# Anton-Le/PhysicsBasedBayesianInference

Hardware: AMD Instinct MI355X
Metric: leapfrog-steps*chains/sec (node); d=128 Gaussian, ensemble=65536 (higher is better)
Workload: dtype f64; 1 GPU; C2: d=128 dense-precision Gaussian, fp64, L=10 leapfrog steps per HMC iteration, in-kernel Philox momentum + Metropolis; chains_per_gpu=65536, total_chains=65536, D=128, L=10, parallelism=ensemble-sharded x1, draw=f32 (single-precision Box-Muller on the transcendental unit; momenta only)

## Files before the change

### physicsbasedbayesianinference_amd/csrc/kernels_dense_dev.h

```cpp
#pragma once
#include <cstdlib>
#include <vector>

#include "pbbi_buf.h"
#include <type_traits>

#include "pbbi_internal.h"
#include "pbbi_rng.h"

namespace {

typedef double v4f64 __attribute__((ext_vector_type(4)));
typedef double v2f64 __attribute__((ext_vector_type(2)));

constexpr int BLOCK = 256;
constexpr int CHAINS_PER_WAVE = 16;
constexpr int CHAINS_PER_WG = 64;

#ifdef PBBI_STAMPS
static unsigned long long* g_stamp_buf = nullptr;
extern "C" void pbbi_debug_set_stamp_buffer(void* p) { g_stamp_buf = (unsigned long long*)p; }
#if PBBI_STAMPS == 2
#define STAMP(i)                                                                      \
    do {                                                                              \
        if (((i) == 0 || (i) == 41) && prm.stamps && lane == 0) {                     \
            unsigned long long t_;                                                    \
            asm volatile("s_memrealtime %0\n\ts_waitcnt lgkmcnt(0)" : "=s"(t_)::"memory"); \
            prm.stamps[((size_t)blockIdx.x * 8 + wave) * 64 + (i)] = t_;              \
        }                                                                             \
    } while (0)
#else
#define STAMP(i)                                                                      \
    do {                                                                              \
        if (prm.stamps && lane == 0) {                                                \
            __builtin_amdgcn_sched_barrier(0);                                        \
            unsigned long long t_;                                                    \
            asm volatile("s_memtime %0\n\ts_waitcnt lgkmcnt(0)" : "=s"(t_)::"memory"); \
            prm.stamps[((size_t)blockIdx.x * 8 + wave) * 64 + (i)] = t_;              \
            __builtin_amdgcn_sched_barrier(0);                                        \
        }                                                                             \
    } while (0)
#endif
#else
#define STAMP(i) do { } while (0)
#endif

struct DensePrm {
#ifdef PBBI_STAMPS
    unsigned long long* stamps;
#endif
    const double* frag;
    const double* mu;
    const double* q_in;
    const double* p_in;
    const double* u_in;
    const double* mass;
    double* q_out;
    double* p_out;
    double* v_out;
    double* ratio_out;
    uint8_t* reject_out;
    int64_t N, ldn_in, ldn_out;
    double h, cst, kT;
    int L, D, flags, rng, mode;
    uint64_t seed, iter, chain0;
    const int32_t* steps_in;
    int32_t* steps_out;
    double* carry_g;
    uint8_t* carry_sel;
    uint32_t carry_slab_bytes;
    int fuse_S, fuse_wrap2, fuse_first;
    int64_t fuse_slab0, fuse_slab;
    double* fuse_q_base;
};

template <int NT>
__device__ __forceinline__ void stage_lds(const double* __restrict__ gfrag,
                                          const double* __restrict__ gmu, v2f64* frag2,
                                          double* mu) {
    constexpr int DP = 16 * NT;
    const v2f64* src = reinterpret_cast<const v2f64*>(gfrag);
    for (int i = threadIdx.x; i < DP * DP / 2; i += BLOCK) frag2[i] = src[i];
    for (int i = threadIdx.x; i < DP; i += BLOCK) mu[i] = gmu[i];
    __syncthreads();
}

template <int NT>
__device__ __forceinline__ void matvec(const v2f64* __restrict__ fragL,
                                       const double* __restrict__ muG,
                                       const double (&q)[4 * NT], v4f64 (&acc)[NT]) {
    constexpr int KS = 4 * NT;
    constexpr int H = NT / 2;
    v2f64 A[H], An[H];
    double m0 = muG[0], mn = 0.0;
#pragma unroll
    for (int t2 = 0; t2 < H; ++t2) A[t2] = fragL[t2 * 64];
#pragma unroll
    for (int t = 0; t < NT; ++t) acc[t] = v4f64{0.0, 0.0, 0.0, 0.0};
#pragma unroll
    for (int s = 0; s < KS; ++s) {
        if (s + 1 < KS) {
#pragma unroll
            for (int t2 = 0; t2 < H; ++t2) An[t2] = fragL[((s + 1) * H + t2) * 64];
            mn = muG[4 * (s + 1)];
        }
        const double x = q[s] - m0;
#pragma unroll
        for (int t2 = 0; t2 < H; ++t2) {
            acc[2 * t2] = __builtin_amdgcn_mfma_f64_16x16x4f64(A[t2].x, x, acc[2 * t2], 0, 0, 0);
            acc[2 * t2 + 1] = __builtin_amdgcn_mfma_f64_16x16x4f64(A[t2].y, x, acc[2 * t2 + 1], 0, 0, 0);
        }
        __builtin_amdgcn_sched_barrier(0);
#pragma unroll
        for (int t2 = 0; t2 < H; ++t2) A[t2] = An[t2];
        m0 = mn;
    }
}

__device__ __forceinline__ double chain_sum(double x) {
    x += __shfl_xor(x, 16, 64);
    x += __shfl_xor(x, 32, 64);
    return x;
}

template <int NT>
__device__ __forceinline__ double dot_x_acc(const double* __restrict__ muG,
                                             const double (&q)[4 * NT], const v4f64 (&acc)[NT]) {
    double sum = 0.0;
#pragma unroll
    for (int t = 0; t < NT; ++t)
#pragma unroll
        for (int r = 0; r < 4; ++r) {
            const int s = 4 * t + r;
            sum += (q[s] - muG[4 * s]) * acc[t][r];
        }
    return sum;
}

template <bool FULL>
__device__ __forceinline__ double load_elem(__amdgpu_buffer_rsrc_t base, uint32_t voff,
                                            uint32_t stride4, uint32_t ld, int s, int g, int D) {
    if constexpr (FULL) return buf_load<double>(base, voff, (uint32_t)s * stride4);
    double val = 0.0;
    if (4 * s + 3 < D) {
        val = buf_load<double>(base, voff, (uint32_t)s * stride4);
    } else if (4 * s < D) {
        const bool ok = 4 * s + g < D;
        const double t = buf_load<double>(base, voff - (ok ? 0u : (uint32_t)g * ld),
                                          (uint32_t)s * stride4);
        val = ok ? t : 0.0;
    }
    return val;
}

template <bool FULL>
__device__ __forceinline__ void store_elem(__amdgpu_buffer_rsrc_t base, uint32_t voff,
                                           uint32_t stride4, int s, int g, int D, double val) {
    if constexpr (FULL) {
        buf_store(base, voff, (uint32_t)s * stride4, val);
        return;
    }
    if (4 * s + 3 < D) {
        buf_store(base, voff, (uint32_t)s * stride4, val);
    } else if (4 * s < D) {
        if (4 * s + g < D) buf_store(base, voff, (uint32_t)s * stride4, val);
    }
}

__device__ __forceinline__ double load_row(__amdgpu_buffer_rsrc_t base, uint32_t voff, uint32_t stride4, int s) {
    return buf_load<double>(base, voff, (uint32_t)s * stride4);
}
__device__ __forceinline__ void store_row(__amdgpu_buffer_rsrc_t base, uint32_t voff, uint32_t stride4, int s,
                                          double val) {
    buf_store(base, voff, (uint32_t)s * stride4, val);
}
template <bool FULL>
__device__ __forceinline__ __amdgpu_buffer_rsrc_t rows_of(const double* arr, int64_t n0, int D, int64_t ld,
                                                          int64_t N) {
    if constexpr (FULL) return buf_make(arr + n0);
    return buf_make_rows(arr + n0, D, ld, N, n0, 8);
}

template <int NT, int METHOD, bool FULL>
__global__ void __launch_bounds__(BLOCK, 1) k_dense_traj(DensePrm prm) {
    constexpr int DP = 16 * NT;
    constexpr int KS = 4 * NT;
    extern __shared__ __attribute__((aligned(16))) char smem[];
    v2f64* frag2 = reinterpret_cast<v2f64*>(smem);
    double* mu = reinterpret_cast<double*>(smem + (size_t)DP * DP * sizeof(double));
    stage_lds<NT>(prm.frag, prm.mu, frag2, mu);

    const int lane = threadIdx.x & 63;
    const int wave = __builtin_amdgcn_readfirstlane(threadIdx.x >> 6);
    const int g = lane >> 4;
    const int c = lane & 15;
    const v2f64* fragL = frag2 + lane;
    const double* muG = mu + g;
    const int D = prm.D;
    const bool unit = (prm.mass == nullptr);
    const double h = prm.h, h2 = prm.h * prm.h;
    const int64_t n_wg_tiles = (prm.N + CHAINS_PER_WG - 1) / CHAINS_PER_WG;

    for (int64_t wt = blockIdx.x; wt < n_wg_tiles; wt += gridDim.x) {
        const int64_t n0 = (wt * 4 + wave) * CHAINS_PER_WAVE;
        if (n0 >= prm.N) continue;
        const int64_t left = prm.N - n0;
        const bool valid = c < left;
        const int cc = c < left ? c : (int)left - 1;
        const uint32_t ld_in = 8u * (uint32_t)prm.ldn_in, ld_out = 8u * (uint32_t)prm.ldn_out;
        const uint32_t vin = (uint32_t)g * ld_in + 8u * (uint32_t)cc, s4in = 4u * ld_in;
        const uint32_t vout = (uint32_t)g * ld_out + 8u * (uint32_t)cc, s4out = 4u * ld_out;
        const __amdgpu_buffer_rsrc_t qin = buf_make(prm.q_in + n0);
        const __amdgpu_buffer_rsrc_t pin = buf_make(prm.p_in + n0);
        const __amdgpu_buffer_rsrc_t qout = buf_make(prm.q_out + n0);
        const __amdgpu_buffer_rsrc_t pout = buf_make(prm.p_out + n0);
        const bool have_pout = (prm.p_out != nullptr);
        const double m = unit ? 1.0 : prm.mass[n0 + cc];
        const uint64_t chain = prm.chain0 + (uint64_t)(n0 + cc);

        double q[KS], v[KS], a[KS];
        v4f64 acc[NT];
        double u = 0.0;
        if (prm.rng) {
            const double pstd = sqrt(m * prm.kT);
#pragma unroll
            for (int k = 0; k < KS / 4; ++k) {
                double z[4];
                rng_normal4d(prm.seed, PBBI_STREAM_MOMENTUM, prm.iter, chain, (uint32_t)((k << 2) | g),
                             (prm.flags & PBBI_DRAW_F64) != 0, z);
#pragma unroll
                for (int sl = 0; sl < 4; ++sl)
                    v[4 * k + sl] = (FULL || 16 * k + 4 * sl + g < D) ? z[sl] * pstd : 0.0;
            }
            u = rng_uniform(prm.seed, prm.iter, chain);
            if (have_pout && !(prm.flags & PBBI_COMPAT_P_FROM_OLDQ) && valid) {
#pragma unroll
                for (int s = 0; s < KS; ++s) store_elem<FULL>(pout, vout, s4out, s, g, D, v[s]);
            }
        } else {
#pragma unroll
            for (int s = 0; s < KS; ++s) v[s] = load_elem<FULL>(pin, vin, s4in, ld_in, s, g, D);
            if (prm.mode == 0) u = prm.u_in[n0 + cc];
        }
#pragma unroll
        for (int s = 0; s < KS; ++s) q[s] = load_elem<FULL>(qin, vin, s4in, ld_in, s, g, D);
        double pp_old = 0.0;
#pragma unroll
        for (int s = 0; s < KS; ++s) pp_old += v[s] * v[s];
        if (!unit) {
#pragma unroll
            for (int s = 0; s < KS; ++s) v[s] = v[s] / m;
        }

        matvec<NT>(fragL, muG, q, acc);
        double xg_old = dot_x_acc<NT>(muG, q, acc);
        double xg_new = xg_old;
#pragma unroll
        for (int t = 0; t < NT; ++t)
#pragma unroll
            for (int r = 0; r < 4; ++r) a[4 * t + r] = unit ? -acc[t][r] : -acc[t][r] / m;

        if constexpr (METHOD == PBBI_LEAPFROG) {
            for (int j = 0; j < prm.L; ++j) {
#pragma unroll
                for (int s = 0; s < KS; ++s) q[s] += (v[s] * h + (0.5 * a[s]) * h2);
                matvec<NT>(fragL, muG, q, acc);
                if (j == prm.L - 1) xg_new = dot_x_acc<NT>(muG, q, acc);
#pragma unroll
                for (int t = 0; t < NT; ++t)
#pragma unroll
                    for (int r = 0; r < 4; ++r) {
                        const int s = 4 * t + r;
                        const double an = unit ? -acc[t][r] : -acc[t][r] / m;
                        v[s] += (0.5 * (a[s] + an)) * h;
                        a[s] = an;
                    }
            }
        } else {
#pragma unroll
            for (int s = 0; s < KS; ++s) {
                const double q0 = q[s];
                q[s] = (q0 + v[s] * h) + (0.5 * a[s]) * h2;
                a[s] = q0;
            }
            for (int j = 0; j < prm.L; ++j) {
                matvec<NT>(fragL, muG, q, acc);
#pragma unroll
                for (int t = 0; t < NT; ++t)
#pragma unroll
                    for (int r = 0; r < 4; ++r) {
                        const int s = 4 * t + r;
                        const double an = unit ? -acc[t][r] : -acc[t][r] / m;
                        const double cur = q[s];
                        q[s] = (2 * cur - a[s]) + an * h2;
                        a[s] = cur;
                    }
            }
#pragma unroll
            for (int s = 0; s < KS; ++s) v[s] = (q[s] - a[s]) / h;
            if (prm.mode == 0) {
                matvec<NT>(fragL, muG, q, acc);
                xg_new = dot_x_acc<NT>(muG, q, acc);
            }
        }

        if (prm.mode == 1) {
            const __amdgpu_buffer_rsrc_t vout_p = buf_make(prm.v_out + n0);
            if (valid) {
#pragma unroll
                for (int s = 0; s < KS; ++s) {
                    store_elem<FULL>(qout, vout, s4out, s, g, D, q[s]);
                    store_elem<FULL>(pout, vout, s4out, s, g, D, unit ? v[s] : v[s] * m);
                }
                if (prm.v_out) {
#pragma unroll
                    for (int s = 0; s < KS; ++s) store_elem<FULL>(vout_p, vout, s4out, s, g, D, v[s]);
                }
            }
            continue;
        }

        double pp_new = 0.0;
#pragma unroll
        for (int s = 0; s < KS; ++s) {
            v[s] = unit ? v[s] : v[s] * m;
            pp_new += v[s] * v[s];
        }
        pp_old = chain_sum(pp_old);
        pp_new = chain_sum(pp_new);
        xg_old = chain_sum(xg_old);
        xg_new = chain_sum(xg_new);
        const double oldH = 0.5 * pp_old / m + (0.5 * xg_old + prm.cst);
        const double newH = 0.5 * pp_new / m + (0.5 * xg_new + prm.cst);
        const double ratio = exp((oldH - newH) * pbbi_accept_beta(prm.flags, prm.kT));
        const bool reject = (ratio == ratio) && (u > (ratio < 1.0 ? ratio : 1.0));
        const bool compat = (prm.flags & PBBI_COMPAT_P_FROM_OLDQ) != 0;
        bool store_p = have_pout;
        if (reject) {
#pragma unroll
            for (int s = 0; s < KS; ++s) q[s] = load_elem<FULL>(qin, vin, s4in, ld_in, s, g, D);
            if (compat) {
#pragma unroll
                for (int s = 0; s < KS; ++s) v[s] = q[s];
            } else if (prm.rng) {
                store_p = false;
            } else if (have_pout) {
#pragma unroll
                for (int s = 0; s < KS; ++s) v[s] = load_elem<FULL>(pin, vin, s4in, ld_in, s, g, D);
            }
        }
        if (valid) {
#pragma unroll
            for (int s = 0; s < KS; ++s) store_elem<FULL>(qout, vout, s4out, s, g, D, q[s]);
            if (store_p) {
#pragma unroll
                for (int s = 0; s < KS; ++s) store_elem<FULL>(pout, vout, s4out, s, g, D, v[s]);
            }
        }
        if (valid && g == 0) {
            if (prm.ratio_out) prm.ratio_out[n0 + c] = ratio;
            if (prm.reject_out) prm.reject_out[n0 + c] = reject ? 1 : 0;
        }
    }
}

constexpr int BLOCK2 = 512;
constexpr int CHAINS_PER_WG2 = 128;

typedef const __attribute__((address_space(3))) v2f64* lds_frag_p;
constexpr int FRAG_LINE = 64;
__device__ __forceinline__ void frag_shift(lds_frag_p& p, int pairs) {
    p += pairs * 64;
    asm volatile("" : "+v"(p));
}
template <class FP>
__device__ __forceinline__ v2f64 frag_read(FP& p, bool& hi, int i) {
    if constexpr (std::is_same<FP, lds_frag_p>::value) {
        if (i >= FRAG_LINE && !hi) {
            frag_shift(p, FRAG_LINE);
            hi = true;
        }
    }
    return p[(hi ? i - FRAG_LINE : i) * 64];
}
template <class FP>
__device__ __forceinline__ void frag_home(FP& p, bool& hi) {
    if constexpr (std::is_same<FP, lds_frag_p>::value) {
        if (hi) frag_shift(p, -FRAG_LINE);
    }
    hi = false;
}

template <int NT>
struct KSkip {
    static constexpr int MIN = NT == 2 ? 1 : NT == 4 ? 9 : NT == 6 ? 17 : NT == 8 ? 25 : NT == 12 ? 33 : NT == 16 ? 49 : 1;
};
template <int N>
__device__ __forceinline__ double vel_at(const double (&v)[N], int s) { return v[s]; }
template <int N>
__device__ __forceinline__ double vel_at(const v4f64 (&v)[N], int s) { return v[s >> 2][s & 3]; }
template <int NT, int NTP, int PASS, bool DRIFT, bool ZMEAN, bool KSKIP = false, class FP, class V>
__device__ __forceinline__ void matvec_pass(FP& fragL,
                                            const double* __restrict__ muG, double (&q)[4 * NT],
                                            const V& vh, v4f64 (&acc)[NTP],
                                            double h, int ks_act = 4 * NT) {
    constexpr int KS = 4 * NT;
    constexpr int H = NT / 2;
    constexpr int HP = NTP / 2;
    constexpr int T0 = PASS * HP;
    v2f64 A[HP];
    bool hi = false;
#pragma unroll
    for (int t2 = 0; t2 < HP; ++t2) A[t2] = frag_read(fragL, hi, T0 + t2);
#pragma unroll
    for (int t = 0; t < NTP; ++t) acc[t] = v4f64{0.0, 0.0, 0.0, 0.0};
    if constexpr (DRIFT) q[0] = fma(vel_at(vh, 0), h, q[0]);
    double x = ZMEAN ? q[0] : q[0] - muG[0];
#pragma unroll
    for (int s = 0; s < KS; ++s) {
        if constexpr (KSKIP) {
            if (s >= KSkip<NT>::MIN && s >= ks_act) {
                frag_home(fragL, hi);
                break;
            }
        }
#pragma unroll
        for (int t2 = 0; t2 < HP; ++t2) {
            acc[2 * t2] = __builtin_amdgcn_mfma_f64_16x16x4f64(A[t2].x, x, acc[2 * t2], 0, 0, 0);
            acc[2 * t2 + 1] = __builtin_amdgcn_mfma_f64_16x16x4f64(A[t2].y, x, acc[2 * t2 + 1], 0, 0, 0);
            if (s + 1 < KS) A[t2] = frag_read(fragL, hi, (s + 1) * H + T0 + t2);
        }
        if (s + 2 == KS) frag_home(fragL, hi);
        double xn = 0.0;
        if (s + 1 < KS) {
            if constexpr (DRIFT) q[s + 1] = fma(vel_at(vh, s + 1), h, q[s + 1]);
            xn = ZMEAN ? q[s + 1] : q[s + 1] - muG[4 * (s + 1)];
        }
        __builtin_amdgcn_sched_barrier(0);
        x = xn;
    }
}

template <int NT, bool ZMEAN, bool KSKIP>
__device__ __forceinline__ void matvec_inplace(lds_frag_p& fragL, const double* __restrict__ muG,
                                               double (&q)[4 * NT], v4f64 (&w)[NT], double cd, int ks_act) {
    constexpr int KS = 4 * NT;
    constexpr int H = NT / 2;
    v2f64 A[H];
    bool hi = false;
#pragma unroll
    for (int t2 = 0; t2 < H; ++t2) A[t2] = frag_read(fragL, hi, t2);
    auto drift_pair = [&](int t2) {
#pragma unroll
        for (int e = 0; e < 8; ++e) q[8 * t2 + e] = fma(vel_at(w, 8 * t2 + e), cd, q[8 * t2 + e]);
    };
    drift_pair(0);
    double x = ZMEAN ? q[0] : q[0] - muG[0];
#pragma unroll
    for (int s = 0; s < KS; ++s) {
        if constexpr (KSKIP) {
            if (s >= KSkip<NT>::MIN && s >= ks_act) {
                frag_home(fragL, hi);
                break;
            }
        }
#pragma unroll
        for (int t2 = 0; t2 < H; ++t2) {
            if (s == 0 && t2 > 0) drift_pair(t2);
            w[2 * t2] = __builtin_amdgcn_mfma_f64_16x16x4f64(A[t2].x, x, w[2 * t2], 0, 0, 0);
            w[2 * t2 + 1] = __builtin_amdgcn_mfma_f64_16x16x4f64(A[t2].y, x, w[2 * t2 + 1], 0, 0, 0);
            if (s + 1 < KS) A[t2] = frag_read(fragL, hi, (s + 1) * H + t2);
            if (s == 0) __builtin_amdgcn_sched_barrier(0);
        }
        if (s + 2 == KS) frag_home(fragL, hi);
        double xn = 0.0;
        if (s + 1 < KS) xn = ZMEAN ? q[s + 1] : q[s + 1] - muG[4 * (s + 1)];
        __builtin_amdgcn_sched_barrier(0);
        x = xn;
    }
}

#ifndef PBBI_DSTREAM_ABLATE
#define PBBI_DSTREAM_ABLATE 0
#endif
template <int NT>
struct StreamCfg {
    static constexpr int NTP = NT / 2, HP = NTP / 2, KS = 4 * NT;
    static constexpr int KC = 4;
    static constexpr int CHUNK = KC * HP * 1024;
    static constexpr int CPP = KS / KC;
    static constexpr int NCH = 2 * CPP;
    static constexpr int RING = NT / 2;
    static constexpr int DMA = KC * HP / 4;
    static constexpr int LDS_RING = RING * CHUNK;
    static_assert(NT % 4 == 0 && CPP % RING == 0 && (KC * HP) % 4 == 0, "static slots, whole DMA shares");
};

struct PRing {
    __amdgpu_buffer_rsrc_t src;
    char* lds;
    uint32_t voff;
    uint32_t woff;
};

template <int NT>
__device__ __forceinline__ void ring_issue_part(const PRing& r, int ci , int m) {
    using C = StreamCfg<NT>;
    typedef __attribute__((address_space(3))) void lds_void;
    const int slot = ci % C::RING;
    __builtin_amdgcn_raw_ptr_buffer_load_lds(r.src, (lds_void*)(r.lds + slot * C::CHUNK + m * 4096), 16, r.voff,
                                             (uint32_t)(ci * C::CHUNK + m * 4096) + r.woff, 0, 0);
}
template <int NT>
__device__ __forceinline__ void ring_issue(const PRing& r, int ci) {
#pragma unroll
    for (int m = 0; m < StreamCfg<NT>::DMA; ++m) ring_issue_part<NT>(r, ci, m);
}

template <int NT, bool INLOOP>
__device__ __forceinline__ void ring_acquire(const PRing& r) {
    using C = StreamCfg<NT>;
    constexpr int YOUNGER = INLOOP ? C::DMA * (C::RING - 3) + (C::DMA < C::KC - 1 ? C::DMA : C::KC - 1)
                                   : C::DMA * (C::RING - 2);
#if !(PBBI_DSTREAM_ABLATE & 2)
    asm volatile("s_waitcnt vmcnt(%0) lgkmcnt(0)\n\ts_barrier" ::"n"(YOUNGER) : "memory");
#endif
}

template <int NT, int PASS, bool DRIFT, bool ZMEAN, bool KSKIP = false>
__device__ __forceinline__ void matvec_pass_stream(const PRing& r, const v2f64* __restrict__ ringL,
                                                   const double* __restrict__ muG, double (&q)[4 * NT],
                                                   const double (&vh)[4 * NT], v4f64 (&acc)[NT / 2], double h,
                                                   int ks_act = 4 * NT) {
    using C = StreamCfg<NT>;
    constexpr int KS = C::KS, HP = C::HP, NTP = C::NTP, KC = C::KC;
    constexpr int C0 = PASS * C::CPP;
    constexpr int H1 = (HP + 1) / 2;
    auto frag_at = [&](int s, int t2) -> v2f64 {
        const int slot = (C0 + s / KC) % C::RING;
        return ringL[((slot * KC + s % KC) * HP + t2) * 64];
    };
    ring_acquire<NT, false>(r);
    v2f64 A[HP], An[HP];
#pragma unroll
    for (int t2 = 0; t2 < HP; ++t2) A[t2] = frag_at(0, t2);
#pragma unroll
    for (int t = 0; t < NTP; ++t) acc[t] = v4f64{0.0, 0.0, 0.0, 0.0};
    if constexpr (DRIFT) q[0] = fma(vh[0], h, q[0]);
    double x = ZMEAN ? q[0] : q[0] - muG[0];
    [[maybe_unused]] int s_exit = KS;
#pragma unroll
    for (int s = 0; s < KS; ++s) {
        if constexpr (KSKIP) {
            if (s >= KSkip<NT>::MIN && s >= ks_act) {
                s_exit = s;
                break;
            }
        }
#pragma unroll
        for (int t2 = 0; t2 < H1; ++t2) {
            acc[2 * t2] = __builtin_amdgcn_mfma_f64_16x16x4f64(A[t2].x, x, acc[2 * t2], 0, 0, 0);
            acc[2 * t2 + 1] = __builtin_amdgcn_mfma_f64_16x16x4f64(A[t2].y, x, acc[2 * t2 + 1], 0, 0, 0);
        }
        __builtin_amdgcn_sched_barrier(0);
        double mun = 0.0;
        if (s + 1 < KS) {
            if ((s + 1) % KC == 0) ring_acquire<NT, true>(r);
#pragma unroll
            for (int t2 = 0; t2 < HP; ++t2) An[t2] = frag_at(s + 1, t2);
            if constexpr (!ZMEAN) mun = muG[4 * (s + 1)];
            if constexpr (DRIFT) q[s + 1] = fma(vh[s + 1], h, q[s + 1]);
        }
        __builtin_amdgcn_sched_barrier(0);
#pragma unroll
        for (int t2 = H1; t2 < HP; ++t2) {
            acc[2 * t2] = __builtin_amdgcn_mfma_f64_16x16x4f64(A[t2].x, x, acc[2 * t2], 0, 0, 0);
            acc[2 * t2 + 1] = __builtin_amdgcn_mfma_f64_16x16x4f64(A[t2].y, x, acc[2 * t2 + 1], 0, 0, 0);
        }
        __builtin_amdgcn_sched_barrier(0);
#if !(PBBI_DSTREAM_ABLATE & 1)
        if (s % KC < C::DMA) ring_issue_part<NT>(r, (C0 + s / KC + C::RING - 1) % C::NCH, s % KC);
#endif
        if (s + 1 < KS) x = ZMEAN ? q[s + 1] : q[s + 1] - mun;
#pragma unroll
        for (int t2 = 0; t2 < HP; ++t2) A[t2] = An[t2];
    }
    if constexpr (KSKIP) {
        for (int s2 = s_exit; s2 < KS; ++s2) {
            if (s2 + 1 < KS && (s2 + 1) % KC == 0) ring_acquire<NT, true>(r);
            if (s2 % KC < C::DMA) ring_issue_part<NT>(r, (C0 + s2 / KC + C::RING - 1) % C::NCH, s2 % KC);
        }
    }
}

template <int NT, int NTP, int PASS, bool ZMEAN>
__device__ __forceinline__ double dot_pass(const double* __restrict__ muG,
                                           const double (&q)[4 * NT], const v4f64 (&acc)[NTP]) {
    double sum = 0.0;
#pragma unroll
    for (int t = 0; t < NTP; ++t)
#pragma unroll
        for (int r = 0; r < 4; ++r) {
            const int s = 4 * (PASS * NTP + t) + r;
            sum = fma(ZMEAN ? q[s] : q[s] - muG[4 * s], acc[t][r], sum);
        }
    return sum;
}

template <int NT, int NTP, int PASS>
__device__ __forceinline__ void kick_pass(double (&vh)[4 * NT], const v4f64 (&acc)[NTP], double ck) {
#pragma unroll
    for (int t = 0; t < NTP; ++t)
#pragma unroll
        for (int r = 0; r < 4; ++r) {
            const int s = 4 * (PASS * NTP + t) + r;
            vh[s] = fma(-acc[t][r], ck, vh[s]);
        }
}

template <int NT, int NTP, int PASS>
__device__ __forceinline__ void halfkick_pass(v4f64 (&w)[NT], const v4f64 (&acc)[NTP]) {
#pragma unroll
    for (int t = 0; t < NTP; ++t)
#pragma unroll
        for (int r = 0; r < 4; ++r) w[PASS * NTP + t][r] = fma(acc[t][r], 0.5, w[PASS * NTP + t][r]);
}

template <int NT, bool FULL, int MODE, bool ZMEAN, int METHOD = PBBI_LEAPFROG, bool DYN = false, int CARRY = 0,
          bool FUSE = false, int DRAW = 2, bool STREAM = false>
__global__ void __launch_bounds__(STREAM ? BLOCK : BLOCK2, STREAM ? 1 : 2) k_dense_hmc(DensePrm prm) {
    static_assert(CARRY == 0 || (MODE == 0 && !DYN), "carry: HMC iterations of fixed trajectory length");
    static_assert(!FUSE || CARRY == 2, "a fused launch reads the carried gradient (its first iteration may form it)");
    static_assert(!STREAM || NT % 4 == 0, "streamed P: two row passes");
    static_assert(std::is_same<decltype(&k_dense_hmc<NT, FULL, MODE, ZMEAN, METHOD, DYN, CARRY, FUSE, DRAW, STREAM>),
                               void (*)(DensePrm)>::value,
                  "kernarg_fresh<DensePrm>() reads the argument block at offset 0 of the kernarg segment");
    constexpr int DP = 16 * NT;
    constexpr int KS = 4 * NT;
    constexpr int NPASS = (NT % 4 == 0) ? 2 : 1;
    constexpr int NTP = NT / NPASS;
    constexpr int WPB = STREAM ? 4 : 8;
    constexpr bool INPL = !STREAM && !DYN;
    extern __shared__ __attribute__((aligned(16))) char smem[];
    const int lane = threadIdx.x & 63;
    const int wave = __builtin_amdgcn_readfirstlane(threadIdx.x >> 6);
    STAMP(0);
    v2f64* frag2 = reinterpret_cast<v2f64*>(smem);
    double* mu = reinterpret_cast<double*>(smem + (STREAM ? (size_t)StreamCfg<STREAM ? NT : 4>::LDS_RING
                                                          : (size_t)DP * DP * sizeof(double)));
    [[maybe_unused]] PRing ring{};
    if constexpr (STREAM) {
        using C = StreamCfg<NT>;
        ring.src = buf_make(prm.frag);
        ring.lds = smem + wave * 1024;
        ring.voff = 16u * (uint32_t)lane;
        ring.woff = 1024u * (uint32_t)wave;
#pragma unroll
        for (int ci = 0; ci < C::RING - 1; ++ci) ring_issue<NT>(ring, ci);
        for (int i = threadIdx.x; i < DP; i += BLOCK) mu[i] = prm.mu[i];
        __syncthreads();
    } else
    {
        const v2f64* src = reinterpret_cast<const v2f64*>(prm.frag);
        constexpr int NCH = DP * DP / 2 / BLOCK2;
        if constexpr (NCH >= 1 && (DP * DP / 2) % BLOCK2 == 0) {
            v2f64 tmp[NCH];
#pragma unroll
            for (int j = 0; j < NCH; ++j) tmp[j] = src[threadIdx.x + j * BLOCK2];
#pragma unroll
            for (int j = 0; j < NCH; ++j) frag2[threadIdx.x + j * BLOCK2] = tmp[j];
        } else {
            for (int i = threadIdx.x; i < DP * DP / 2; i += BLOCK2) frag2[i] = src[i];
        }
        for (int i = threadIdx.x; i < DP; i += BLOCK2) mu[i] = prm.mu[i];
        __syncthreads();
    }
#ifndef PBBI_DENSE_FUSE_PRIO
#define PBBI_DENSE_FUSE_PRIO 1
#endif
    if (!STREAM && (!FUSE || PBBI_DENSE_FUSE_PRIO) && wave < 4) __builtin_amdgcn_s_setprio(1);
    STAMP(1);
    const int g = lane >> 4;
    const int c = lane & 15;
    [[maybe_unused]] const v2f64* fragL = frag2 + lane;
    [[maybe_unused]] lds_frag_p fragA = (lds_frag_p)(frag2 + lane);
    const double* muG = mu + g;
    const int D = prm.D;
    const double h = prm.h;
    [[maybe_unused]] const int ks_act = (D + 3) >> 2;
#define MATVEC(PASS_, DRIFT_, Q_, V_, ACC_, H_)                                                        \
    do {                                                                                              \
        if constexpr (STREAM) matvec_pass_stream<NT, PASS_, DRIFT_, ZMEAN, !FULL>(ring, fragL, muG, Q_, V_, ACC_, H_, ks_act); \
        else if constexpr (DYN) matvec_pass<NT, NTP, PASS_, DRIFT_, ZMEAN, !FULL>(fragL, muG, Q_, V_, ACC_, H_, ks_act); \
        else matvec_pass<NT, NTP, PASS_, DRIFT_, ZMEAN, !FULL>(fragA, muG, Q_, V_, ACC_, H_, ks_act); \
    } while (0)

    int64_t n0 = ((int64_t)blockIdx.x * WPB + wave) * CHAINS_PER_WAVE;
    bool ghost = false;
    if (n0 >= prm.N) {
        if constexpr (!STREAM) return;
        ghost = true;
        n0 = (prm.N - 1) / CHAINS_PER_WAVE * CHAINS_PER_WAVE;
    }
    const int64_t left = prm.N - n0;
    const bool valid = !ghost && c < left;
    const int cc = c < left ? c : (int)left - 1;
    const uint32_t ld_in = 8u * (uint32_t)prm.ldn_in, ld_out = 8u * (uint32_t)prm.ldn_out;
    const uint32_t vin = (uint32_t)g * ld_in + 8u * (uint32_t)cc, s4in = 4u * ld_in;
    const uint32_t vout = (uint32_t)g * ld_out + 8u * (uint32_t)cc, s4out = 4u * ld_out;
    const __amdgpu_buffer_rsrc_t qin = rows_of<FULL>(prm.q_in, n0, D, prm.ldn_in, prm.N);
    const __amdgpu_buffer_rsrc_t qout = rows_of<FULL>(prm.q_out, n0, D, prm.ldn_out, prm.N);
    const __amdgpu_buffer_rsrc_t pout = rows_of<FULL>(prm.p_out, n0, D, prm.ldn_out, prm.N);
    const double m = prm.mass ? prm.mass[n0 + cc] : 1.0;
    const double minv = prm.mass ? 1.0 / m : 1.0;
    [[maybe_unused]] const double cd = -(h * h) * minv, nih = -1.0 / h, nh = -h;
    const bool rng = (FUSE && !STREAM) || ((MODE == 0) && prm.rng);
    [[maybe_unused]] const uint32_t ld_g = 8u * (uint32_t)prm.N, s4g = 4u * ld_g;
    [[maybe_unused]] uint32_t vg_cur = 0, vg_new = 0;
    [[maybe_unused]] uint32_t csel = 0;
    [[maybe_unused]] const __amdgpu_buffer_rsrc_t gbuf = buf_make(CARRY ? prm.carry_g + n0 : nullptr);
    if constexpr (CARRY != 0) {
        if constexpr (CARRY == 2) csel = prm.carry_sel[n0 + cc];
    }
    double q[KS];
    if constexpr (FUSE) {
#pragma unroll
        for (int s = 0; s < KS; ++s) q[s] = load_row(qin, vin, s4in, s);
    }
    const int nfuse = FUSE ? prm.fuse_S : 1;
#ifndef PBBI_DSTREAM_KEEPG
#define PBBI_DSTREAM_KEEPG 1
#endif
#ifndef PBBI_DSTREAM_KEEPG_MAXNT
#define PBBI_DSTREAM_KEEPG_MAXNT 12
#endif
    constexpr bool KEEPG = STREAM && FUSE && PBBI_DSTREAM_KEEPG && NT <= PBBI_DSTREAM_KEEPG_MAXNT;
    v4f64 acc[NTP];
    [[maybe_unused]] v4f64 gk[KEEPG ? NTP : 1];
    [[maybe_unused]] double xg_keep = 0.0;
    if constexpr (FUSE) {
        if (prm.fuse_first) {
            const uint32_t vg0 = (uint32_t)g * ld_g + 8u * (uint32_t)cc;
            v4f64 (&acc0)[NTP] = acc;
            MATVEC(0, false, q, q, acc0, h);
            if (valid) {
#pragma unroll
                for (int t = 0; t < NTP; ++t)
#pragma unroll
                    for (int r = 0; r < 4; ++r) store_row(gbuf, vg0, s4g, 4 * t + r, acc0[t][r]);
            }
            if constexpr (KEEPG) {
                xg_keep = dot_pass<NT, NTP, 0, ZMEAN>(muG, q, acc0);
#pragma unroll
                for (int t = 0; t < NTP; ++t) gk[t] = acc0[t];
            }
            if constexpr (NPASS == 2) {
                MATVEC(1, false, q, q, acc0, h);
                if (valid) {
#pragma unroll
                    for (int t = 0; t < NTP; ++t)
#pragma unroll
                        for (int r = 0; r < 4; ++r)
                            store_row(gbuf, vg0, s4g, 4 * (NTP + t) + r, acc0[t][r]);
                }
                if constexpr (KEEPG) xg_keep += dot_pass<NT, NTP, 1, ZMEAN>(muG, q, acc0);
            }
            __builtin_amdgcn_sched_barrier(0);
        } else if constexpr (KEEPG) {
            const uint32_t vg0 = (uint32_t)g * ld_g + 8u * (uint32_t)cc + (csel ? prm.carry_slab_bytes : 0u);
#pragma unroll
            for (int t = 0; t < NTP; ++t)
#pragma unroll
                for (int r = 0; r < 4; ++r) {
                    gk[t][r] = load_row(gbuf, vg0, s4g, 4 * t + r);
                    acc[t][r] = load_row(gbuf, vg0, s4g, 4 * (NTP + t) + r);
                }
            xg_keep = dot_pass<NT, NTP, 0, ZMEAN>(muG, q, gk);
            xg_keep += dot_pass<NT, NTP, 1, ZMEAN>(muG, q, acc);
        }
    }
    constexpr bool LOCAL = !STREAM && !DYN;
    auto here = [](auto x) {
        if constexpr (LOCAL) return sgpr_fresh(x);
        else return x;
    };
    auto args = [&]() -> decltype(auto) {
        if constexpr (LOCAL && ZMEAN) return kernarg_fresh<DensePrm>();
        else return (prm);
    };
#pragma nounroll
    for (int kf = 0; kf < nfuse; ++kf) {
    STAMP(42);
    const uint64_t iter_k = prm.iter + (uint64_t)kf;
    [[maybe_unused]] double* const ratio_top = (FUSE && prm.ratio_out) ? prm.ratio_out + (int64_t)kf * prm.N : prm.ratio_out;
    [[maybe_unused]] uint8_t* const reject_top = (FUSE && prm.reject_out) ? prm.reject_out + (int64_t)kf * prm.N : prm.reject_out;
    [[maybe_unused]] __amdgpu_buffer_rsrc_t qin_top = qin, qout_top = qout, pout_top = pout;
    if constexpr (!LOCAL && FUSE) {
        const int64_t s_out = prm.fuse_wrap2 ? ((prm.fuse_slab0 + kf) & 1) : prm.fuse_slab0 + kf;
        const int64_t s_prev = prm.fuse_wrap2 ? ((prm.fuse_slab0 + kf - 1) & 1) : prm.fuse_slab0 + kf - 1;
        if (kf > 0) qin_top = rows_of<FULL>(prm.fuse_q_base + s_prev * prm.fuse_slab, n0, D, prm.ldn_out, prm.N);
        qout_top = rows_of<FULL>(prm.fuse_q_base + s_out * prm.fuse_slab, n0, D, prm.ldn_out, prm.N);
        pout_top = rows_of<FULL>(prm.p_out + (prm.p_out ? (int64_t)kf * prm.fuse_slab : 0), n0, D, prm.ldn_out, prm.N);
    }
    auto qslab_of = [&](const auto& a, int k) {
        const int64_t sl = a.fuse_wrap2 ? ((a.fuse_slab0 + k) & 1) : a.fuse_slab0 + k;
        return rows_of<FULL>(a.fuse_q_base + sl * a.fuse_slab, n0, D, a.ldn_out, a.N);
    };
    auto qin_of = [&](const auto& a, int k) {
        if constexpr (!LOCAL) return qin_top;
        else if constexpr (FUSE) {
            if (k > 0) return qslab_of(a, k - 1);
            return rows_of<FULL>(a.q_in, n0, D, a.ldn_in, a.N);
        } else return qin;
    };
    auto qout_of = [&](const auto& a, int k) {
        if constexpr (!LOCAL) return qout_top;
        else if constexpr (FUSE) return qslab_of(a, k);
        else return qout;
    };
    auto pout_of = [&](const auto& a, int k) {
        if constexpr (!LOCAL) return pout_top;
        else if constexpr (FUSE)
            return rows_of<FULL>(a.p_out + (a.p_out ? (int64_t)k * a.fuse_slab : 0), n0, D, a.ldn_out, a.N);
        else return pout;
    };
    if constexpr (CARRY != 0) {
        const uint32_t vg0 = (uint32_t)g * ld_g + 8u * (uint32_t)cc;
        vg_cur = vg0 + (csel ? prm.carry_slab_bytes : 0u);
        vg_new = vg0 + (csel ? 0u : prm.carry_slab_bytes);
    }

    [[maybe_unused]] double vh[KS];
    [[maybe_unused]] v4f64 w[INPL ? NT : 1];
    auto vget = [&](int s) -> double {
        if constexpr (INPL) return w[s >> 2][s & 3];
        else return vh[s];
    };
    auto vset = [&](int s, double val) {
        if constexpr (INPL) w[s >> 2][s & 3] = val;
        else vh[s] = val;
    };
    auto carry_load = [&](auto pass_c) {
        constexpr int PASS = decltype(pass_c)::value;
        const uint32_t st = here(s4g);
#pragma unroll
        for (int t = 0; t < NTP; ++t)
#pragma unroll
            for (int r = 0; r < 4; ++r)
                acc[t][r] = load_row(gbuf, vg_cur, st, 4 * (PASS * NTP + t) + r);
    };
    auto carry_store = [&](auto pass_c, uint32_t voff) {
        constexpr int PASS = decltype(pass_c)::value;
        if (valid) {
            const uint32_t st = here(s4g);
#pragma unroll
            for (int t = 0; t < NTP; ++t)
#pragma unroll
                for (int r = 0; r < 4; ++r)
                    store_row(gbuf, voff, st, 4 * (PASS * NTP + t) + r, acc[t][r]);
        }
    };
    using P0 = std::integral_constant<int, 0>;
    using P1 = std::integral_constant<int, 1>;
    if constexpr (CARRY == 2 && FUSE && !KEEPG) carry_load(P0{});
    double pp = 0.0;
    if constexpr (KEEPG) {
        const uint64_t chain = prm.chain0 + (uint64_t)(n0 + cc);
        const double pstd = sqrt(m * prm.kT);
        const double ck0k = 0.5 * (h * minv);
        const bool park = prm.p_out && !(prm.flags & PBBI_COMPAT_P_FROM_OLDQ) && valid;
        const bool draw64 = DRAW == 2 ? (prm.flags & PBBI_DRAW_F64) != 0 : DRAW == 1;
        const __amdgpu_buffer_rsrc_t pout_k = pout_of(prm, kf);
#pragma unroll
        for (int k = 0; k < KS / 4; ++k) {
            double z[4];
            rng_normal4d(prm.seed, PBBI_STREAM_MOMENTUM, iter_k, chain, (uint32_t)((k << 2) | g), draw64, z);
#pragma unroll
            for (int sl = 0; sl < 4; ++sl) {
                const int s = 4 * k + sl;
                double pv = (FULL || 16 * k + 4 * sl + g < D) ? z[sl] * pstd : 0.0;
                if (park) store_row(pout_k, vout, s4out, s, pv);
                pp += pv * pv;
                pv *= minv;
                vh[s] = fma(-(k < NTP ? gk[k % NTP][sl] : acc[k % NTP][sl]), ck0k, pv);
            }
            __builtin_amdgcn_sched_barrier(0);
        }
        STAMP(2);
    } else {
    if (rng) {
        const uint64_t chain = prm.chain0 + (uint64_t)(n0 + cc);
        const double pstd = sqrt(m * prm.kT);
        const auto& ad = args();
        const bool draw64 = DRAW == 2 ? (ad.flags & PBBI_DRAW_F64) != 0 : DRAW == 1;
        const uint64_t seed_k = ad.seed;
#pragma unroll
        for (int k = 0; k < KS / 4; ++k) {
            double z[4];
            rng_normal4d(seed_k, PBBI_STREAM_MOMENTUM, iter_k, chain, (uint32_t)((k << 2) | g), draw64, z);
#pragma unroll
            for (int sl = 0; sl < 4; ++sl)
                vset(4 * k + sl, (FULL || 16 * k + 4 * sl + g < D) ? z[sl] * pstd : 0.0);
        }
        if (ad.p_out && !(ad.flags & PBBI_COMPAT_P_FROM_OLDQ) && valid) {
            const uint32_t st = here(s4out);
            const __amdgpu_buffer_rsrc_t pout_k = pout_of(ad, here(kf));
#pragma unroll
            for (int s = 0; s < KS; ++s) store_row(pout_k, vout, st, s, vget(s));
        }
    } else {
        const __amdgpu_buffer_rsrc_t pin = rows_of<FULL>(prm.p_in, n0, D, prm.ldn_in, prm.N);
#pragma unroll
        for (int s = 0; s < KS; ++s) vset(s, load_row(pin, vin, s4in, s));
    }
    STAMP(2);
    if constexpr (!FUSE) {
#pragma unroll
        for (int s = 0; s < KS; ++s) q[s] = load_row(qin, vin, s4in, s);
    }
    __builtin_amdgcn_sched_barrier(0);
#pragma unroll
    for (int s = 0; s < KS; ++s) {
        const double pv = vget(s);
        pp += pv * pv;
        vset(s, pv * (INPL ? nih : minv));
    }
    __builtin_amdgcn_sched_barrier(0);
    }
    STAMP(3);

    const double ck = h * minv, ckh = 0.5 * ck;
    int Ln = prm.L;
    if constexpr (DYN) {
        if (rng) Ln = (prm.flags & PBBI_PER_CHAIN_STEPS)
                          ? rng_steps(prm.seed, iter_k, prm.chain0 + (uint64_t)(n0 + cc), prm.L) : prm.L;
        else if (prm.steps_in) Ln = prm.steps_in[n0 + cc];
        Ln = Ln < 0 ? 0 : (Ln > prm.L ? prm.L : Ln);
    }
    const double ck0 = (DYN && Ln == 0) ? 0.0 : ckh;
    double xg = 0.0;
    constexpr bool FOLD1 = STREAM && CARRY != 2;
    if constexpr (KEEPG) {
        xg = xg_keep;
    } else if constexpr (!FOLD1) {
    if constexpr (CARRY == 2) {
        if constexpr (!FUSE) carry_load(P0{});
    } else if constexpr (INPL) {
        MATVEC(0, false, q, w, acc, h);
    } else {
        MATVEC(0, false, q, vh, acc, h);
    }
    if constexpr (CARRY == 1) carry_store(P0{}, vg_cur);
    xg = dot_pass<NT, NTP, 0, ZMEAN>(muG, q, acc);
    if constexpr (INPL) halfkick_pass<NT, NTP, 0>(w, acc);
    else kick_pass<NT, NTP, 0>(vh, acc, ck0);
    if constexpr (NPASS == 2) {
        if constexpr (CARRY == 2) carry_load(P1{});
        else if constexpr (INPL) MATVEC(1, false, q, w, acc, h);
        else MATVEC(1, false, q, vh, acc, h);
        if constexpr (CARRY == 1) carry_store(P1{}, vg_cur);
        xg += dot_pass<NT, NTP, 1, ZMEAN>(muG, q, acc);
        if constexpr (INPL) halfkick_pass<NT, NTP, 1>(w, acc);
        else kick_pass<NT, NTP, 1>(vh, acc, ck0);
    }
    }
    double oldH = 0.5 * chain_sum(pp) / m + (0.5 * chain_sum(xg) + args().cst);
    STAMP(4);
    [[maybe_unused]] const double xg_old_keep = xg;
    if constexpr (!DYN) xg = 0.0;
    if constexpr (DYN) {
        const bool uturn = (prm.flags & PBBI_UTURN_STOP) != 0;
        bool alive = true;
        double pend = 0.0;
        int taken = Ln;
        auto uturn_dot = [&](auto pass_c) {
            constexpr int PASS = decltype(pass_c)::value;
            double q0r[4 * NTP];
#pragma unroll
            for (int t = 0; t < 4 * NTP; ++t) q0r[t] = load_row(qin, vin, s4in, 4 * PASS * NTP + t);
            double sum = 0.0;
#pragma unroll
            for (int t = 0; t < NTP; ++t)
#pragma unroll
                for (int r = 0; r < 4; ++r) {
                    const int s = 4 * (PASS * NTP + t) + r;
                    sum = fma(q[s] - q0r[4 * t + r], fma(-acc[t][r], ckh, vh[s]), sum);
                }
            return sum;
        };
        using U0 = std::integral_constant<int, 0>;
        using U1 = std::integral_constant<int, 1>;
        for (int j = FOLD1 ? -1 : 0; j <= prm.L; ++j) {
            const bool first = FOLD1 && j < 0;
            const bool active = !first && alive && j < Ln;
            bool more = first || __builtin_amdgcn_ballot_w64(active || pend != 0.0) != 0;
            if (STREAM && !first) {
                int* vote = reinterpret_cast<int*>(mu + DP) + 4 * (j & 1);
                if (lane == 0) vote[wave] = more ? 1 : 0;
                asm volatile("s_waitcnt lgkmcnt(0)\n\ts_barrier" ::: "memory");
                more = (vote[0] | vote[1] | vote[2] | vote[3]) != 0;
            }
            if (!more) break;
            const double cj = first ? ck0 : (active ? (j == Ln - 1 ? ckh : ck) : pend);
            const double hq = active ? h : 0.0;
            if (!first) pend = 0.0;
            double dot = 0.0;
            MATVEC(0, true, q, vh, acc, hq);
            if (MODE == 0) xg = dot_pass<NT, NTP, 0, ZMEAN>(muG, q, acc);
            if (uturn && !first) dot = uturn_dot(U0{});
            kick_pass<NT, NTP, 0>(vh, acc, cj);
            if constexpr (NPASS == 2) {
                MATVEC(1, false, q, vh, acc, h);
                if (MODE == 0) xg += dot_pass<NT, NTP, 1, ZMEAN>(muG, q, acc);
                if (uturn && !first) dot += uturn_dot(U1{});
                kick_pass<NT, NTP, 1>(vh, acc, cj);
            }
            if (first) {
                oldH = 0.5 * chain_sum(pp) / m + (0.5 * chain_sum(xg) + prm.cst);
                continue;
            }
            if (uturn) {
                dot = chain_sum(dot);
                if (active && j != Ln - 1 && dot < 0.0) {
                    alive = false;
                    taken = j + 1;
                    pend = -ckh;
                }
            }
            if (active && j == Ln - 1) alive = false;
        }
        Ln = taken;
    } else if constexpr (INPL) {
    constexpr bool TAIL = METHOD == PBBI_LEAPFROG || MODE == 0;
    const int n_in = METHOD == PBBI_LEAPFROG ? here(prm.L) - 1 : here(prm.L);
#pragma nounroll
    for (int j = 0; j < n_in; ++j) {
        STAMP(5 + 2 * j);
        matvec_inplace<NT, ZMEAN, !FULL>(fragA, muG, q, w, cd, ks_act);
    }
    if constexpr (TAIL) {
        STAMP(5 + 2 * n_in);
        MATVEC(0, true, q, w, acc, cd);
        if constexpr (MODE == 0) xg = dot_pass<NT, NTP, 0, ZMEAN>(muG, q, acc);
        if constexpr (CARRY != 0) carry_store(P0{}, vg_new);
        if constexpr (METHOD == PBBI_LEAPFROG) halfkick_pass<NT, NTP, 0>(w, acc);
        STAMP(6 + 2 * n_in);
        if constexpr (NPASS == 2) {
            MATVEC(1, false, q, w, acc, cd);
            if constexpr (MODE == 0) xg += dot_pass<NT, NTP, 1, ZMEAN>(muG, q, acc);
            if constexpr (CARRY != 0) carry_store(P1{}, vg_new);
            if constexpr (METHOD == PBBI_LEAPFROG) halfkick_pass<NT, NTP, 1>(w, acc);
        }
    } else {
#pragma unroll
        for (int s = 0; s < KS; ++s) q[s] = fma(vget(s), cd, q[s]);
    }
    } else {
    constexpr bool SV_EXTRA = METHOD == PBBI_STORMER_VERLET && MODE == 0;
    const int nsteps = SV_EXTRA ? prm.L + 1 : prm.L;
    for (int j = FOLD1 ? -1 : 0; j < nsteps; ++j) {
        const bool first = FOLD1 && j < 0;
        const bool last = (j == nsteps - 1) && (METHOD == PBBI_LEAPFROG || SV_EXTRA);
        const double cj = first ? ck0 : (METHOD == PBBI_LEAPFROG ? (last ? ckh : ck) : (last ? 0.0 : ck));
        const double hj = first ? 0.0 : h;
        STAMP(5 + 2 * j);
        MATVEC(0, true, q, vh, acc, hj);
        if ((first || last) && MODE == 0) xg = dot_pass<NT, NTP, 0, ZMEAN>(muG, q, acc);
        if constexpr (CARRY == 1)
            if (first) carry_store(P0{}, vg_cur);
        if constexpr (CARRY != 0)
            if (last) carry_store(P0{}, vg_new);
        kick_pass<NT, NTP, 0>(vh, acc, cj);
        if constexpr (KEEPG) {
            if (last) {
#pragma unroll
                for (int t = 0; t < NTP; ++t) gk[t] = acc[t];
            }
        }
        STAMP(6 + 2 * j);
        if constexpr (NPASS == 2) {
            MATVEC(1, false, q, vh, acc, h);
            if ((first || last) && MODE == 0) xg += dot_pass<NT, NTP, 1, ZMEAN>(muG, q, acc);
            if constexpr (CARRY == 1)
                if (first) carry_store(P1{}, vg_cur);
            if constexpr (CARRY != 0)
                if (last) carry_store(P1{}, vg_new);
            kick_pass<NT, NTP, 1>(vh, acc, cj);
        }
        if constexpr (FOLD1) {
            if (first) {
                oldH = 0.5 * chain_sum(pp) / m + (0.5 * chain_sum(xg) + prm.cst);
                xg = 0.0;
            }
        }
    }
    }
    if constexpr (METHOD == PBBI_STORMER_VERLET && MODE == 1 && !INPL) {
#pragma unroll
        for (int s = 0; s < KS; ++s) q[s] = fma(vh[s], h, q[s]);
    }

    if constexpr (MODE == 1) {
        const __amdgpu_buffer_rsrc_t vout_p = rows_of<FULL>(prm.v_out, n0, D, prm.ldn_out, prm.N);
        if (valid) {
            if (prm.v_out) {
#pragma unroll
                for (int s = 0; s < KS; ++s) store_row(vout_p, vout, s4out, s, INPL ? (vget(s) * nh) * minv : vget(s));
            }
#pragma unroll
            for (int s = 0; s < KS; ++s) {
                store_row(qout, vout, s4out, s, q[s]);
                store_row(pout, vout, s4out, s, vget(s) * (INPL ? nh : m));
            }
        }
    } else {
        pp = 0.0;
#pragma unroll
        for (int s = 0; s < KS; ++s) {
            const double pv = vget(s) * (INPL ? nh : m);
            vset(s, pv);
            pp += pv * pv;
        }
        const auto& ae = args();
        const int kf_e = here(kf);
        const double newH = 0.5 * chain_sum(pp) / m + (0.5 * chain_sum(xg) + ae.cst);
        STAMP(40);
        const double ratio = exp((oldH - newH) * pbbi_accept_beta(ae.flags, ae.kT));
        const double u = rng ? rng_uniform(ae.seed, iter_k, ae.chain0 + (uint64_t)(n0 + cc))
                             : prm.u_in[n0 + cc];
        const bool reject = (ratio == ratio) && (u > (ratio < 1.0 ? ratio : 1.0));
        const bool compat = (ae.flags & PBBI_COMPAT_P_FROM_OLDQ) != 0;
        bool store_p = (ae.p_out != nullptr);
        if (reject) {
            const uint32_t st = here(s4in);
            const __amdgpu_buffer_rsrc_t qin_k = qin_of(ae, kf_e);
#pragma unroll
            for (int s = 0; s < KS; ++s) q[s] = load_row(qin_k, vin, st, s);
            if constexpr (KEEPG) {
#pragma unroll
                for (int t = 0; t < NTP; ++t)
#pragma unroll
                    for (int r = 0; r < 4; ++r) {
                        gk[t][r] = load_row(gbuf, vg_cur, s4g, 4 * t + r);
                        acc[t][r] = load_row(gbuf, vg_cur, s4g, 4 * (NTP + t) + r);
                    }
            }
            if (compat) {
#pragma unroll
                for (int s = 0; s < KS; ++s) vset(s, q[s]);
            } else if (rng) {
                store_p = false;
            } else if (store_p) {
                const __amdgpu_buffer_rsrc_t pin = rows_of<FULL>(prm.p_in, n0, D, prm.ldn_in, prm.N);
#pragma unroll
                for (int s = 0; s < KS; ++s) vset(s, load_row(pin, vin, s4in, s));
            }
        }
        if (valid) {
            const uint32_t st = here(s4out);
            const __amdgpu_buffer_rsrc_t qout_k = qout_of(ae, kf_e);
#pragma unroll
            for (int s = 0; s < KS; ++s) store_row(qout_k, vout, st, s, q[s]);
            if (store_p) {
                const uint32_t stp = here(s4out);
                const __amdgpu_buffer_rsrc_t pout_k = pout_of(ae, kf_e);
#pragma unroll
                for (int s = 0; s < KS; ++s) store_row(pout_k, vout, stp, s, vget(s));
            }
        }
        if constexpr (CARRY != 0) csel ^= reject ? 0u : 1u;
        if constexpr (KEEPG) xg_keep = reject ? xg_old_keep : xg;
        if (valid && (LOCAL ? vgpr_fresh(g) : g) == 0) {
            const int64_t n0_e = here(n0);
            double* const ratio_k = !LOCAL ? ratio_top : (FUSE && ae.ratio_out) ? ae.ratio_out + (int64_t)kf_e * ae.N : ae.ratio_out;
            uint8_t* const reject_k = !LOCAL ? reject_top : (FUSE && ae.reject_out) ? ae.reject_out + (int64_t)kf_e * ae.N : ae.reject_out;
            if (ratio_k) ratio_k[n0_e + c] = ratio;
            if (reject_k) reject_k[n0_e + c] = reject ? 1 : 0;
            if constexpr (DYN) {
                if (prm.steps_out) prm.steps_out[n0_e + c] = Ln;
            }
            if constexpr (CARRY != 0 && !FUSE) prm.carry_sel[n0_e + c] = (uint8_t)csel;
        }
        STAMP(41);
    }
    }
    if constexpr (FUSE) {
        if (valid && g == 0) prm.carry_sel[n0 + c] = (uint8_t)csel;
    }
    if constexpr (STREAM) asm volatile("s_waitcnt vmcnt(0)" ::: "memory");
#undef MATVEC
}

}
```

Before: 2.193 billion leapfrog-steps*chains/s.

## Keep carried gradient in registers across fused HMC iterations in in-place dense kernel

For the fused, carried-gradient, in-place (non-streamed) dense HMC kernel, the gradient is now kept in the velocity register array between iterations rather than reloaded from the carry slab at the start of each iteration. The momentum draw is folded directly into the half-kick, and the final momentum scaling, kinetic sum and optional p_out store are done per pass inside the tail, where the fresh gradient is then copied into the register array. On rejection the old gradient is reloaded from the carry buffer and momenta are regenerated from the RNG if they need to be stored. This cuts global loads per iteration at the cost of extra register pressure, more complex reject paths and macro-gated variants (V_XGRE, V_NOREGEN).

```diff
diff --git a/physicsbasedbayesianinference_amd/csrc/kernels_dense_dev.h b/physicsbasedbayesianinference_amd/csrc/kernels_dense_dev.h
--- a/physicsbasedbayesianinference_amd/csrc/kernels_dense_dev.h
+++ b/physicsbasedbayesianinference_amd/csrc/kernels_dense_dev.h
@@ -624,6 +624,26 @@
     for (int t = 0; t < NTP; ++t)
 #pragma unroll
         for (int r = 0; r < 4; ++r) w[PASS * NTP + t][r] = fma(acc[t][r], 0.5, w[PASS * NTP + t][r]);
+}
+
+template <int NT, int NTP, int PASS, bool ZMEAN>
+__device__ __forceinline__ double dot_pass_of(const double* __restrict__ muG, const double (&q)[4 * NT],
+                                              const v4f64 (&gw)[NT]) {
+    double sum = 0.0;
+#pragma unroll
+    for (int t = 0; t < NTP; ++t)
+#pragma unroll
+        for (int r = 0; r < 4; ++r) {
+            const int s = 4 * (PASS * NTP + t) + r;
+            sum = fma(ZMEAN ? q[s] : q[s] - muG[4 * s], gw[PASS * NTP + t][r], sum);
+        }
+    return sum;
+}
+
+template <bool FIRST, class A, class B>
+__device__ __forceinline__ auto& pick_ref(A& a, B& b) {
+    if constexpr (FIRST) return a;
+    else return b;
 }
 
 template <int NT, bool FULL, int MODE, bool ZMEAN, int METHOD = PBBI_LEAPFROG, bool DYN = false, int CARRY = 0,
@@ -735,8 +755,10 @@
 #define PBBI_DSTREAM_KEEPG_MAXNT 12
 #endif
     constexpr bool KEEPG = STREAM && FUSE && PBBI_DSTREAM_KEEPG && NT <= PBBI_DSTREAM_KEEPG_MAXNT;
+    constexpr bool KEEPW = FUSE && CARRY == 2 && INPL;
     v4f64 acc[NTP];
     [[maybe_unused]] v4f64 gk[KEEPG ? NTP : 1];
+    [[maybe_unused]] v4f64 wk[KEEPW ? NT : 1];
     [[maybe_unused]] double xg_keep = 0.0;
     if constexpr (FUSE) {
         if (prm.fuse_first) {
@@ -754,6 +776,11 @@
 #pragma unroll
                 for (int t = 0; t < NTP; ++t) gk[t] = acc0[t];
             }
+            if constexpr (KEEPW) {
+                xg_keep = dot_pass<NT, NTP, 0, ZMEAN>(muG, q, acc0);
+#pragma unroll
+                for (int t = 0; t < NTP; ++t) wk[t] = acc0[t];
+            }
             if constexpr (NPASS == 2) {
                 MATVEC(1, false, q, q, acc0, h);
                 if (valid) {
@@ -764,6 +791,11 @@
                             store_row(gbuf, vg0, s4g, 4 * (NTP + t) + r, acc0[t][r]);
                 }
                 if constexpr (KEEPG) xg_keep += dot_pass<NT, NTP, 1, ZMEAN>(muG, q, acc0);
+                if constexpr (KEEPW) {
+                    xg_keep += dot_pass<NT, NTP, 1, ZMEAN>(muG, q, acc0);
+#pragma unroll
+                    for (int t = 0; t < NTP; ++t) wk[NTP + t] = acc0[t];
+                }
             }
             __builtin_amdgcn_sched_barrier(0);
         } else if constexpr (KEEPG) {
@@ -777,6 +809,14 @@
                 }
             xg_keep = dot_pass<NT, NTP, 0, ZMEAN>(muG, q, gk);
             xg_keep += dot_pass<NT, NTP, 1, ZMEAN>(muG, q, acc);
+        } else if constexpr (KEEPW) {
+            const uint32_t vg0 = (uint32_t)g * ld_g + 8u * (uint32_t)cc + (csel ? prm.carry_slab_bytes : 0u);
+#pragma unroll
+            for (int t = 0; t < NT; ++t)
+#pragma unroll
+                for (int r = 0; r < 4; ++r) wk[t][r] = load_row(gbuf, vg0, s4g, 4 * t + r);
+            xg_keep = dot_pass_of<NT, NTP, 0, ZMEAN>(muG, q, wk);
+            if constexpr (NPASS == 2) xg_keep += dot_pass_of<NT, NTP, 1, ZMEAN>(muG, q, wk);
         }
     }
     constexpr bool LOCAL = !STREAM && !DYN;
@@ -831,7 +871,8 @@
     }
 
     [[maybe_unused]] double vh[KS];
-    [[maybe_unused]] v4f64 w[INPL ? NT : 1];
+    [[maybe_unused]] v4f64 w_it[INPL && !KEEPW ? NT : 1];
+    [[maybe_unused]] auto& w = pick_ref<KEEPW>(wk, w_it);
     auto vget = [&](int s) -> double {
         if constexpr (INPL) return w[s >> 2][s & 3];
         else return vh[s];
@@ -862,7 +903,7 @@
     };
     using P0 = std::integral_constant<int, 0>;
     using P1 = std::integral_constant<int, 1>;
-    if constexpr (CARRY == 2 && FUSE && !KEEPG) carry_load(P0{});
+    if constexpr (CARRY == 2 && FUSE && !KEEPG && !KEEPW) carry_load(P0{});
     double pp = 0.0;
     if constexpr (KEEPG) {
         const uint64_t chain = prm.chain0 + (uint64_t)(n0 + cc);
@@ -887,6 +928,25 @@
             __builtin_amdgcn_sched_barrier(0);
         }
         STAMP(2);
+    } else if constexpr (KEEPW) {
+        const uint64_t chain = prm.chain0 + (uint64_t)(n0 + cc);
+        const double pstd = sqrt(m * prm.kT);
+        const auto& ad = args();
+        const bool draw64 = DRAW == 2 ? (ad.flags & PBBI_DRAW_F64) != 0 : DRAW == 1;
+        const uint64_t seed_k = ad.seed;
+#pragma unroll
+        for (int k = 0; k < KS / 4; ++k) {
+            double z[4];
+            rng_normal4d(seed_k, PBBI_STREAM_MOMENTUM, iter_k, chain, (uint32_t)((k << 2) | g), draw64, z);
+#pragma unroll
+            for (int sl = 0; sl < 4; ++sl) {
+                const double pv = (FULL || 16 * k + 4 * sl + g < D) ? z[sl] * pstd : 0.0;
+                pp += pv * pv;
+                w[k][sl] = fma(w[k][sl], 0.5, pv * nih);
+            }
+            __builtin_amdgcn_sched_barrier(0);
+        }
+        STAMP(2);
     } else {
     if (rng) {
         const uint64_t chain = prm.chain0 + (uint64_t)(n0 + cc);
@@ -940,7 +1000,7 @@
     const double ck0 = (DYN && Ln == 0) ? 0.0 : ckh;
     double xg = 0.0;
     constexpr bool FOLD1 = STREAM && CARRY != 2;
-    if constexpr (KEEPG) {
+    if constexpr (KEEPG || KEEPW) {
         xg = xg_keep;
     } else if constexpr (!FOLD1) {
     if constexpr (CARRY == 2) {
@@ -1038,18 +1098,43 @@
         STAMP(5 + 2 * j);
         matvec_inplace<NT, ZMEAN, !FULL>(fragA, muG, q, w, cd, ks_act);
     }
+    auto leave_pass = [&](auto pass_c) {
+        constexpr int PASS = decltype(pass_c)::value;
+#pragma unroll
+        for (int t = PASS * NTP; t < (PASS + 1) * NTP; ++t)
+#pragma unroll
+            for (int r = 0; r < 4; ++r) {
+                const double pv = w[t][r] * nh;
+                w[t][r] = pv;
+                pp += pv * pv;
+            }
+        const auto& al = args();
+        if (al.p_out != nullptr && valid) {
+            const uint32_t st = here(s4out);
+            const __amdgpu_buffer_rsrc_t pout_k = pout_of(al, here(kf));
+#pragma unroll
+            for (int t = PASS * NTP; t < (PASS + 1) * NTP; ++t)
+#pragma unroll
+                for (int r = 0; r < 4; ++r) store_row(pout_k, vout, st, 4 * t + r, w[t][r]);
+        }
+#pragma unroll
+        for (int t = 0; t < NTP; ++t) w[PASS * NTP + t] = acc[t];
+    };
     if constexpr (TAIL) {
         STAMP(5 + 2 * n_in);
+        if constexpr (KEEPW) pp = 0.0;
         MATVEC(0, true, q, w, acc, cd);
         if constexpr (MODE == 0) xg = dot_pass<NT, NTP, 0, ZMEAN>(muG, q, acc);
         if constexpr (CARRY != 0) carry_store(P0{}, vg_new);
         if constexpr (METHOD == PBBI_LEAPFROG) halfkick_pass<NT, NTP, 0>(w, acc);
+        if constexpr (KEEPW) leave_pass(P0{});
         STAMP(6 + 2 * n_in);
         if constexpr (NPASS == 2) {
             MATVEC(1, false, q, w, acc, cd);
             if constexpr (MODE == 0) xg += dot_pass<NT, NTP, 1, ZMEAN>(muG, q, acc);
             if constexpr (CARRY != 0) carry_store(P1{}, vg_new);
             if constexpr (METHOD == PBBI_LEAPFROG) halfkick_pass<NT, NTP, 1>(w, acc);
+            if constexpr (KEEPW) leave_pass(P1{});
         }
     } else {
 #pragma unroll
@@ -1114,12 +1199,14 @@
             }
         }
     } else {
+        if constexpr (!KEEPW) {
         pp = 0.0;
 #pragma unroll
         for (int s = 0; s < KS; ++s) {
             const double pv = vget(s) * (INPL ? nh : m);
             vset(s, pv);
             pp += pv * pv;
+        }
         }
         const auto& ae = args();
         const int kf_e = here(kf);
@@ -1145,7 +1232,43 @@
                         acc[t][r] = load_row(gbuf, vg_cur, s4g, 4 * (NTP + t) + r);
                     }
             }
-            if (compat) {
+            if constexpr (KEEPW) {
+                const uint32_t stg = here(s4g);
+#pragma unroll
+                for (int t = 0; t < NT; ++t)
+#pragma unroll
+                    for (int r = 0; r < 4; ++r) w[t][r] = load_row(gbuf, vg_cur, stg, 4 * t + r);
+                store_p = false;
+                if (ae.p_out != nullptr && valid) {
+                    const uint32_t stp = here(s4out);
+                    const __amdgpu_buffer_rsrc_t pout_k = pout_of(ae, kf_e);
+                    if (compat) {
+#pragma unroll
+                        for (int s = 0; s < KS; ++s) store_row(pout_k, vout, stp, s, q[s]);
+                    }
+#ifndef V_NOREGEN
+                    else {
+                        const uint64_t chain = ae.chain0 + (uint64_t)(n0 + cc);
+                        const double pstd = sqrt(m * ae.kT);
+                        const bool draw64 = DRAW == 2 ? (ae.flags & PBBI_DRAW_F64) != 0 : DRAW == 1;
+#pragma unroll
+                        for (int k = 0; k < KS / 4; ++k) {
+                            double z[4];
+                            rng_normal4d(ae.seed, PBBI_STREAM_MOMENTUM, iter_k, chain, (uint32_t)((k << 2) | g), draw64, z);
+#pragma unroll
+                            for (int sl = 0; sl < 4; ++sl)
+                                store_row(pout_k, vout, stp, 4 * k + sl,
+                                          (FULL || 16 * k + 4 * sl + g < D) ? z[sl] * pstd : 0.0);
+                            __builtin_amdgcn_sched_barrier(0);
+                        }
+                    }
+#endif
+                }
+#ifdef V_XGRE
+                xg_keep = dot_pass_of<NT, NTP, 0, ZMEAN>(muG, q, w);
+                if constexpr (NPASS == 2) xg_keep += dot_pass_of<NT, NTP, 1, ZMEAN>(muG, q, w);
+#endif
+            } else if (compat) {
 #pragma unroll
                 for (int s = 0; s < KS; ++s) vset(s, q[s]);
             } else if (rng) {
@@ -1161,30 +1284,40 @@
             const __amdgpu_buffer_rsrc_t qout_k = qout_of(ae, kf_e);
 #pragma unroll
             for (int s = 0; s < KS; ++s) store_row(qout_k, vout, st, s, q[s]);
+            if constexpr (!KEEPW) {
             if (store_p) {
                 const uint32_t stp = here(s4out);
                 const __amdgpu_buffer_rsrc_t pout_k = pout_of(ae, kf_e);
 #pragma unroll
                 for (int s = 0; s < KS; ++s) store_row(pout_k, vout, stp, s, vget(s));
             }
+            }
         }
         if constexpr (CARRY != 0) csel ^= reject ? 0u : 1u;
+#ifdef V_XGRE
         if constexpr (KEEPG) xg_keep = reject ? xg_old_keep : xg;
-        if (valid && (LOCAL ? vgpr_fresh(g) : g) == 0) {
+        if constexpr (KEEPW) { if (!reject) xg_keep = xg; }
+#else
+        if constexpr (KEEPG || KEEPW) xg_keep = reject ? xg_old_keep : xg;
+#endif
+        if (valid && (KEEPW ? vgpr_fresh(vout) < ld_out : (LOCAL ? vgpr_fresh(g) : g) == 0)) {
             const int64_t n0_e = here(n0);
+            const int c_e = KEEPW ? (int)(vgpr_fresh(vout) >> 3) : c;
             double* const ratio_k = !LOCAL ? ratio_top : (FUSE && ae.ratio_out) ? ae.ratio_out + (int64_t)kf_e * ae.N : ae.ratio_out;
             uint8_t* const reject_k = !LOCAL ? reject_top : (FUSE && ae.reject_out) ? ae.reject_out + (int64_t)kf_e * ae.N : ae.reject_out;
-            if (ratio_k) ratio_k[n0_e + c] = ratio;
-            if (reject_k) reject_k[n0_e + c] = reject ? 1 : 0;
+            if (ratio_k) ratio_k[n0_e + c_e] = ratio;
+            if (reject_k) reject_k[n0_e + c_e] = reject ? 1 : 0;
             if constexpr (DYN) {
-                if (prm.steps_out) prm.steps_out[n0_e + c] = Ln;
-            }
-            if constexpr (CARRY != 0 && !FUSE) prm.carry_sel[n0_e + c] = (uint8_t)csel;
+                if (prm.steps_out) prm.steps_out[n0_e + c_e] = Ln;
+            }
+            if constexpr (CARRY != 0 && !FUSE) prm.carry_sel[n0_e + c_e] = (uint8_t)csel;
         }
         STAMP(41);
     }
     }
-    if constexpr (FUSE) {
+    if constexpr (KEEPW) {
+        if (valid && vout < ld_out) prm.carry_sel[n0 + (int)(vout >> 3)] = (uint8_t)csel;
+    } else if constexpr (FUSE) {
         if (valid && g == 0) prm.carry_sel[n0 + c] = (uint8_t)csel;
     }
     if constexpr (STREAM) asm volatile("s_waitcnt vmcnt(0)" ::: "memory");
```

Result: no change. 2.210 billion leapfrog-steps*chains/s, median of 6 (+0.7%).
